# NirajNair/vector-indexer

Hardware: AMD Instinct MI355X
Metric: QPS at recall@10>=0.95 (IVF search, SIFT1M-shaped) (higher is better)
Workload: dtype f32; 1 GPU; IVF search N=1000000 D=128 nlist=4096 nprobe=32 k=10 nq/step=10000 (BASELINE configs[1]); nprobe=32, index_centroids=4094, parallelism=1 GPU

## Files before the change

### vector-indexer_amd/csrc/mfma_bf16.hpp

```cpp
#pragma once
#include <hip/hip_runtime.h>

#include <cmath>
#include <cstdint>

namespace vi {

typedef __bf16 bf16x8 __attribute__((ext_vector_type(8)));
typedef float f32x16 __attribute__((ext_vector_type(16)));
typedef __attribute__((address_space(3))) void *lds_ptr_t;

__device__ __forceinline__ float min3_raw(float a, float b, float c) {
  float d;
  asm("v_min3_f32 %0, %1, %2, %3" : "=v"(d) : "v"(a), "v"(b), "v"(c));
  return d;
}
__device__ __forceinline__ float opaque_neg_inf() {
  float v;
  asm("v_mov_b32 %0, 0xff800000" : "=v"(v));
  return v;
}
__device__ __forceinline__ void tile_min_level1(const f32x16 &a, float ninf, float (&p)[8]) {
#pragma unroll
  for (int i = 0; i < 8; ++i) p[i] = __builtin_amdgcn_fmed3f(ninf, a[2 * i], a[2 * i + 1]);
}
__device__ __forceinline__ float tile_min_level2(const float (&p)[8]) {
  const float m0 = min3_raw(p[0], p[1], p[2]), m1 = min3_raw(p[3], p[4], p[5]), m2 = min3_raw(p[6], p[7], p[7]);
  return min3_raw(m0, m1, m2);
}
__device__ __forceinline__ float tile_min(const f32x16 &a) {
  float p[8];
  tile_min_level1(a, opaque_neg_inf(), p);
  return tile_min_level2(p);
}
#define VI_TOP4(v)                             \
  {                                            \
    T3 = __builtin_amdgcn_fmed3f(T2, T3, v);   \
    T2 = __builtin_amdgcn_fmed3f(T1, T2, v);   \
    T1 = __builtin_amdgcn_fmed3f(T0, T1, v);   \
    T0 = min3_raw(T0, v, v);                   \
  }

__device__ __forceinline__ uint32_t bf16_rn(float x) {
  const uint32_t b = __float_as_uint(x);
  return (b + 0x7FFFu + ((b >> 16) & 1u)) >> 16;
}
__device__ __forceinline__ void split_pair(float x0, float x1, uint32_t &hi, uint32_t &lo) {
  const uint32_t h0 = bf16_rn(x0), h1 = bf16_rn(x1);
  const float r0 = x0 - __uint_as_float(h0 << 16), r1 = x1 - __uint_as_float(h1 << 16);
  hi = h0 | (h1 << 16);
  lo = bf16_rn(r0) | (bf16_rn(r1) << 16);
}
__device__ __forceinline__ void split8(const float4 &lo4, const float4 &hi4, float scale, uint4 &hi, uint4 &lo) {
  split_pair(scale * lo4.x, scale * lo4.y, hi.x, lo.x);
  split_pair(scale * lo4.z, scale * lo4.w, hi.y, lo.y);
  split_pair(scale * hi4.x, scale * hi4.y, hi.z, lo.z);
  split_pair(scale * hi4.z, scale * hi4.w, hi.w, lo.w);
}

template <int NG, int WAVES = 4>
__device__ __forceinline__ void tile_dma_image(float *tile, const float4 *src, const float *xn, int wave, int lane) {
#pragma unroll
  for (int i = 0; i < 2 * NG / WAVES; ++i) {
    const int piece = wave + WAVES * i;
    __builtin_amdgcn_global_load_lds(src + piece * 64 + lane, (lds_ptr_t)(tile + piece * 256), 16, 0, 0);
  }
  if (wave == 0) __builtin_amdgcn_global_load_lds(xn + lane, (lds_ptr_t)(tile + 2 * NG * 256), 4, 0, 0);
}

__device__ __forceinline__ void glds16_asm(const void *gsrc, float *lds_dst) {
  unsigned keep;
  const unsigned dst = (unsigned)__builtin_amdgcn_readfirstlane((int)(size_t)(lds_ptr_t)lds_dst);
  asm volatile("s_mov_b32 %0, m0\n\ts_mov_b32 m0, %2\n\ts_nop 0\n\tglobal_load_lds_dwordx4 %1, off\n\ts_mov_b32 m0, %0"
               : "=&s"(keep) : "v"(gsrc), "s"(dst) : "memory");
}
__device__ __forceinline__ void glds16_at(const void *gsrc, unsigned lds_addr) {
  unsigned keep;
  const unsigned dst = (unsigned)__builtin_amdgcn_readfirstlane((int)lds_addr);
  asm volatile("s_mov_b32 %0, m0\n\ts_mov_b32 m0, %2\n\ts_nop 0\n\tglobal_load_lds_dwordx4 %1, off\n\ts_mov_b32 m0, %0"
               : "=&s"(keep) : "v"(gsrc), "s"(dst) : "memory");
}
__device__ __forceinline__ void glds4_at(const void *gsrc, unsigned lds_addr) {
  unsigned keep;
  const unsigned dst = (unsigned)__builtin_amdgcn_readfirstlane((int)lds_addr);
  asm volatile("s_mov_b32 %0, m0\n\ts_mov_b32 m0, %2\n\ts_nop 0\n\tglobal_load_lds_dword %1, off\n\ts_mov_b32 m0, %0"
               : "=&s"(keep) : "v"(gsrc), "s"(dst) : "memory");
}
__device__ __forceinline__ void glds4_asm(const void *gsrc, float *lds_dst) {
  unsigned keep;
  const unsigned dst = (unsigned)__builtin_amdgcn_readfirstlane((int)(size_t)(lds_ptr_t)lds_dst);
  asm volatile("s_mov_b32 %0, m0\n\ts_mov_b32 m0, %2\n\ts_nop 0\n\tglobal_load_lds_dword %1, off\n\ts_mov_b32 m0, %0"
               : "=&s"(keep) : "v"(gsrc), "s"(dst) : "memory");
}

template <int NG, int WAVES = 4>
__device__ __forceinline__ void tile_dma_image_asm(float *tile, const float4 *src, const float *xn, int wave, int lane) {
#pragma unroll
  for (int i = 0; i < 2 * NG / WAVES; ++i) {
    const int piece = wave + WAVES * i;
    glds16_asm(src + piece * 64 + lane, tile + piece * 256);
  }
  if (wave == 0) glds4_asm(xn + lane, tile + 2 * NG * 256);
}

}
```

### vector-indexer_amd/csrc/rank_stream.hip

```cpp
#include <hip/hip_runtime.h>

#include <algorithm>
#include <cmath>
#include <cstdint>
#include <cstdio>
#include <cstdlib>
#include <vector>

#include "common.hpp"
#include "mfma_bf16.hpp"
#include "rank_stream.hpp"

namespace vi {
namespace {

constexpr int kWave = 64;
#ifdef VI_STREAM_PROF_BUILD
constexpr bool kStreamProf = true;
#else
constexpr bool kStreamProf = false;
#endif

typedef int i32x4 __attribute__((ext_vector_type(4)));
typedef int i32x16 __attribute__((ext_vector_type(16)));

template <int NC, int NA, class N4>
struct TileRegs {
  uint4 a[NC * NA];
  N4 n[4];
};

template <int IP, int NC, int NA, class N4, class N>
__device__ __forceinline__ void load_tile(TileRegs<NC, NA, N4> &t, const uint4 *img, const N *norm, uint32_t blk, uint32_t half, int il,
                                          int h) {
  const uint4 *ap = img + ((size_t)blk * (NC * 2 * IP) + h) * kWave + 32u * half + il;
#pragma unroll
  for (int c = 0; c < NC; ++c)
#pragma unroll
    for (int p = 0; p < NA; ++p) t.a[c * NA + p] = ap[(c * IP + p) * 2 * kWave];
  const N *np = norm + (size_t)blk * kWave + 32u * half + 4 * h;
#pragma unroll
  for (int q4 = 0; q4 < 4; ++q4) t.n[q4] = *reinterpret_cast<const N4 *>(np + 8 * q4);
}

template <int R>
struct StreamLayout {
  static constexpr int RP = R <= 2 ? 2 : R <= 4 ? 4 : R <= 8 ? 8 : R <= 16 ? 16 : 32;
  static_assert(R <= 32, "row too long");
  __device__ static __forceinline__ uint32_t swz(uint32_t pc, uint32_t q) {
    if constexpr (RP >= 16) return pc ^ (q & 15u);
    else return pc ^ ((q / (16u / RP)) & (uint32_t)(RP - 1));
  }
};

struct ItemRaw {
  uint4 d;
  uint32_t qid;
  uint32_t rec[2];
};
struct ItemRegs {
  uint32_t nqi, blk00, ntiles, rec0;
};

template <int NC, int NA, class N4>
__device__ __forceinline__ void tile_landed(const TileRegs<NC, NA, N4> &t) {
#pragma unroll
  for (int i = 0; i < NC * NA; ++i) asm volatile("" ::"v"(t.a[i].x), "v"(t.a[i].y), "v"(t.a[i].z), "v"(t.a[i].w));
#pragma unroll
  for (int q4 = 0; q4 < 4; ++q4) asm volatile("" ::"v"(t.n[q4].x), "v"(t.n[q4].y), "v"(t.n[q4].z), "v"(t.n[q4].w));
  __builtin_amdgcn_sched_barrier(0);
}

__device__ __forceinline__ void wait_vmcnt(uint32_t n) {
  switch (n) {
    case 1: asm volatile("s_waitcnt vmcnt(1)" ::: "memory"); break;
    case 2: asm volatile("s_waitcnt vmcnt(2)" ::: "memory"); break;
    case 3: asm volatile("s_waitcnt vmcnt(3)" ::: "memory"); break;
    case 4: asm volatile("s_waitcnt vmcnt(4)" ::: "memory"); break;
    case 5: asm volatile("s_waitcnt vmcnt(5)" ::: "memory"); break;
    case 6: asm volatile("s_waitcnt vmcnt(6)" ::: "memory"); break;
    case 7: asm volatile("s_waitcnt vmcnt(7)" ::: "memory"); break;
    case 8: asm volatile("s_waitcnt vmcnt(8)" ::: "memory"); break;
    default: asm volatile("s_waitcnt vmcnt(0)" ::: "memory"); break;
  }
}

__device__ __forceinline__ uint32_t queue_pop_asm(uint32_t *counter) {
  uint32_t ret;
  const uint32_t one = 1u;
  asm volatile("global_atomic_add %0, %1, %2, off sc0" : "=v"(ret) : "v"(counter), "v"(one) : "memory");
  return ret;
}

__device__ __forceinline__ void item_landed(const ItemRaw &r) {
  asm volatile("" ::"v"(r.d.x), "v"(r.d.y), "v"(r.d.z), "v"(r.d.w), "v"(r.qid), "v"(r.rec[0]), "v"(r.rec[1]));
  __builtin_amdgcn_sched_barrier(0);
}

__device__ __forceinline__ int tile_min_i32(const i32x16 &a) {
  int m[8];
#pragma unroll
  for (int i = 0; i < 8; ++i) m[i] = min(a[2 * i], a[2 * i + 1]);
  return min(min(min(m[0], m[1]), min(m[2], m[3])), min(min(m[4], m[5]), min(m[6], m[7])));
}


template <int RANK, bool QLO>
struct Bf16Form {
  static_assert(RANK == 2 || QLO, "bf16 x 3 needs the queries' lo plane");
  using Args = RankStreamArgs;
  using Norm4 = float4;
  using Frag = bf16x8;
  using Acc = f32x16;
  static constexpr int NA = RANK == 1 ? 2 : 1;
  static constexpr int NP = QLO ? 2 : 1;
  static constexpr int IP = 2;
  static constexpr bool kHooks = true;
  static constexpr int kRank = RANK;
  static constexpr bool kQlo = QLO;
  static constexpr const char *kName = "rank kernel";
  __device__ static __forceinline__ const float *norms(const Args &a) { return a.xnorm; }
  __device__ static __forceinline__ uint32_t xmode(const Args &a) { return a.xmode; }
  __device__ static __forceinline__ unsigned long long *prof(const Args &a) { return a.prof; }
  template <class T>
  __device__ static __forceinline__ Acc chunk(Acc acc, const T &t, int c, const Frag (&b)[NP]) {
    const bf16x8 ah = __builtin_bit_cast(bf16x8, t.a[c * NA]);
    acc = __builtin_amdgcn_mfma_f32_32x32x16_bf16(ah, b[0], acc, 0, 0, 0);
    if constexpr (QLO) acc = __builtin_amdgcn_mfma_f32_32x32x16_bf16(ah, b[NP - 1], acc, 0, 0, 0);
    if constexpr (RANK == 1) {
      const bf16x8 al = __builtin_bit_cast(bf16x8, t.a[c * NA + 1]);
      acc = __builtin_amdgcn_mfma_f32_32x32x16_bf16(al, b[0], acc, 0, 0, 0);
    }
    return acc;
  }
  __device__ static __forceinline__ float minimum(const Acc &acc) { return tile_min(acc); }
};

struct I8Form {
  using Args = RankStreamI8Args;
  using Norm4 = int4;
  using Frag = i32x4;
  using Acc = i32x16;
  static constexpr int NA = 1, NP = 1, IP = 1;
  static constexpr bool kHooks = false;
  static constexpr const char *kName = "int8 rank kernel";
  __device__ static __forceinline__ const int *norms(const Args &a) { return a.hnorm; }
  __device__ static __forceinline__ uint32_t xmode(const Args &) { return 0u; }
  __device__ static __forceinline__ unsigned long long *prof(const Args &) { return nullptr; }
  template <class T>
  __device__ static __forceinline__ Acc chunk(Acc acc, const T &t, int c, const Frag (&b)[NP]) {
    return __builtin_amdgcn_mfma_i32_32x32x32_i8(__builtin_bit_cast(i32x4, t.a[c]), b[0], acc, 0, 0, 0);
  }
  __device__ static __forceinline__ float minimum(const Acc &acc) { return (float)(2 * tile_min_i32(acc)); }
};

template <class F, int NC, int NU>
struct StreamShape {
  static constexpr int GQ = 32 * NU;
  using L = StreamLayout<2 * NC * F::NP>;
  static constexpr int IMG = GQ * L::RP * 16;
  static constexpr bool DB = IMG <= 32 * 1024;
  static constexpr size_t kLds = (size_t)IMG * (DB ? 2 : 1) + 2 * (size_t)NU * 1024 + 16;
};

template <class F, int NC, int NU>
__device__ __forceinline__ void rank_stream_body(typename F::Args a) {
  using S = StreamShape<F, NC, NU>;
  using L = typename S::L;
  using Tile = TileRegs<NC, F::NA, typename F::Norm4>;
  using Frag = typename F::Frag;
  constexpr int NP = F::NP;
  constexpr int GQ = S::GQ;
  constexpr int NR = NU / 4;
  constexpr int RP = L::RP;
  constexpr int RPI = 64 / RP;
  constexpr int IPW = GQ * RP / 256;
  constexpr int IMG = S::IMG;
  constexpr bool DB = S::DB;
  extern __shared__ __attribute__((aligned(16))) float s_mem[];
  float *s_T = s_mem + (DB ? 2 : 1) * (IMG / 4);
  uint32_t *s_idx = reinterpret_cast<uint32_t *>(s_T + 2 * 4 * NU * kWave);
  const int lane = threadIdx.x & (kWave - 1), wave = threadIdx.x >> 6;
  const int j = lane & 31, h = lane >> 5;
  const unsigned lds_q = (unsigned)(size_t)(lds_ptr_t)s_mem;
  auto load = [&](Tile &t, uint32_t blk, uint32_t half) { load_tile<F::IP>(t, a.img, F::norms(a), blk, half, j, h); };

  auto request_item = [&](uint32_t it, ItemRaw &r) {
    r.d = make_uint4(0u, 0u, 0u, 0u); r.qid = ~0u; r.rec[0] = ~0u; r.rec[1] = ~0u;
    if (it >= a.nitems) return;
    r.d = a.sdesc[it];
    if ((uint32_t)lane < (uint32_t)(GQ / 4)) r.qid = a.qcol[(size_t)it * GQ + (uint32_t)wave * (GQ / 4) + (uint32_t)lane];
#pragma unroll
    for (int k = 0; k < NR; ++k) r.rec[k] = a.grec[(size_t)it * GQ + 32u * ((uint32_t)wave + 4u * k) + (uint32_t)j];
  };
  auto decode_item = [&](const ItemRaw &r) {
    ItemRegs o;
    o.nqi = (uint32_t)__builtin_amdgcn_readfirstlane((int)r.d.x);
    o.blk00 = (uint32_t)__builtin_amdgcn_readfirstlane((int)r.d.y);
    o.ntiles = (uint32_t)__builtin_amdgcn_readfirstlane((int)r.d.z);
    o.rec0 = (uint32_t)__builtin_amdgcn_readfirstlane((int)r.d.w);
    return o;
  };
  auto gather = [&](uint32_t buf, uint32_t nq_item, uint32_t my_qid) {
    if (F::xmode(a) & 32u) return;
    uint32_t lo = (uint32_t)lane;
    asm volatile("" : "+v"(lo));
    uint32_t qids[IPW];
#pragma unroll
    for (int i = 0; i < IPW; ++i) qids[i] = (uint32_t)__shfl((int)my_qid, (int)(RPI * i + lo / RP));
#pragma unroll
    for (int i = 0; i < IPW; ++i) {
      const uint32_t row0 = (uint32_t)wave * (GQ / 4) + (uint32_t)(RPI * i);
      if (row0 < nq_item) {
        const uint32_t pc = L::swz(lo % RP, row0 + lo / RP);
        if (qids[i] != ~0u && pc < 2u * NC * NP)
          glds16_at(a.qimg + (size_t)qids[i] * (NC * 2 * F::IP) + pc, lds_q + buf * (uint32_t)IMG + row0 * RP * 16u);
      }
    }
  };

  const unsigned long long rt_begin = F::prof(a) ? __builtin_amdgcn_s_memrealtime() : 0ull;
  constexpr uint32_t kQueues = 8;
  auto queue_range = [&](uint32_t q, uint32_t &lo, uint32_t &hi) {
    lo = (uint32_t)(((uint64_t)a.nitems * q) / kQueues);
    hi = (uint32_t)(((uint64_t)a.nitems * (q + 1)) / kQueues);
  };
  uint32_t my_queue = blockIdx.x % kQueues;
  auto resolve = [&](uint32_t popped) {
    for (uint32_t tries = 0; tries < kQueues; ++tries) {
      uint32_t lo, hi;
      queue_range(my_queue, lo, hi);
      if (popped < hi - lo) return lo + popped;
      my_queue = (my_queue + 1) % kQueues;
      if (tries + 1 < kQueues) popped = atomicAdd(a.queue + 32 * my_queue, 1u);
    }
    return a.nitems;
  };
  const bool fixed = (F::xmode(a) & 64u) != 0u;
  if (threadIdx.x == 0) {
#pragma unroll
    for (uint32_t k = 0; k < 2; ++k) s_idx[k] = fixed ? blockIdx.x + k * gridDim.x : resolve(atomicAdd(a.queue + 32 * my_queue, 1u));
  }
  __syncthreads();
  uint32_t cur = (uint32_t)__builtin_amdgcn_readfirstlane((int)s_idx[0]), nxt = (uint32_t)__builtin_amdgcn_readfirstlane((int)s_idx[1]);
  ItemRaw rc, rn;
  request_item(cur, rc);
  request_item(nxt, rn);
  ItemRegs ic = decode_item(rc);
  Tile ta, tb;
  if ((uint32_t)wave < ic.ntiles) load(ta, ic.blk00 + ((uint32_t)wave >> 1), (uint32_t)wave & 1u);
  gather(0u, ic.nqi, rc.qid);
  asm volatile("s_waitcnt vmcnt(0)" ::: "memory");
  __syncthreads();
  tile_landed(ta);

  unsigned long long pt[16] = {0, 0, 0, 0, 0, 0, 0, 0, 0, 0, 0, 0, 0, 0, 0, 0};
  const bool prof = kStreamProf && F::prof(a) != nullptr && wave == 0;
  unsigned long long tk = prof ? __builtin_amdgcn_s_memtime() : 0ull;
  const unsigned long long tk_begin = tk;
  auto lap = [&](int slot) {
    if (prof) {
      const unsigned long long now = __builtin_amdgcn_s_memtime();
      pt[slot] += now - tk;
      tk = now;
    }
  };
  uint32_t buf = 0;
  uint32_t par = 0;
  uint32_t n_items = 0;
  const uint32_t lane_row = ((uint32_t)j * RP + L::swz(0u, (uint32_t)j)) * 16u;
  while (cur < a.nitems) {
    uint32_t after = ~0u;
    ItemRegs in{0u, 0u, 0u, 0u};
    auto last_step = [&](Tile &spare) {
      in = decode_item(rn);
      if ((uint32_t)wave < in.ntiles) load(spare, in.blk00 + ((uint32_t)wave >> 1), (uint32_t)wave & 1u);
      if (threadIdx.x == 0) after = fixed ? nxt + gridDim.x : queue_pop_asm(a.queue + 32 * my_queue);
      if (DB) gather(buf ^ 1u, in.nqi, rn.qid);
    };
    const uint32_t nqi = ic.nqi, nu = (ic.nqi + 31u) >> 5, ntiles = ic.ntiles, blk00 = ic.blk00;
    const char *img_at = reinterpret_cast<const char *>(s_mem) + (DB ? buf * (uint32_t)IMG : 0u);
    auto frag = [&](int c, int p, int u) {
      const uint32_t pc = (uint32_t)(p * 2 * NC + 2 * c) + (uint32_t)h;
      return __builtin_bit_cast(Frag, *reinterpret_cast<const uint4 *>(img_at + ((lane_row ^ (pc << 4)) + (uint32_t)(32 * u * RP * 16))));
    };

    float T[NU];
    float4 pend[NU];
#pragma unroll
    for (int u = 0; u < NU; ++u) {
      T[u] = INFINITY;
      pend[u] = make_float4(INFINITY, INFINITY, INFINITY, INFINITY);
    }
    const uint32_t bi = ic.rec0 * (2u * GQ) + (uint32_t)GQ * (uint32_t)h + (uint32_t)j;

    constexpr int kPF = 4;
    auto step = [&](const Tile &t, uint32_t i, bool last) {
      typename F::Acc nrm;
#pragma unroll
      for (int q4 = 0; q4 < 4; ++q4) {
        nrm[4 * q4 + 0] = t.n[q4].x; nrm[4 * q4 + 1] = t.n[q4].y; nrm[4 * q4 + 2] = t.n[q4].z; nrm[4 * q4 + 3] = t.n[q4].w;
      }
      Frag ring[kPF][NP];
      auto fetch = [&](int s) {
        const int u = (s / NC) < NU - 1 ? (s / NC) : NU - 1, c = s % NC;
#pragma unroll
        for (int p = 0; p < NP; ++p) ring[s % kPF][p] = frag(c, p, u);
      };
#pragma unroll
      for (int s0 = 0; s0 < kPF; ++s0) fetch(s0);
      const uint32_t ci = i & 3u;
#pragma unroll
      for (int u = 0; u < NU; ++u) {
        if ((uint32_t)u < nu) {
          typename F::Acc acc = nrm;
#pragma unroll
          for (int c = 0; c < NC; ++c) {
            const int sp = u * NC + c;
            __builtin_amdgcn_sched_barrier(0);
            acc = F::chunk(acc, t, c, ring[sp % kPF]);
            __builtin_amdgcn_sched_barrier(0);
            fetch(sp + kPF);
          }
          if (!(F::xmode(a) & 2u)) {
            const float m = F::minimum(acc);
            T[u] = min3_raw(T[u], m, m);
            pend[u].x = ci == 0u ? m : pend[u].x;
            pend[u].y = ci == 1u ? m : pend[u].y;
            pend[u].z = ci == 2u ? m : pend[u].z;
            pend[u].w = ci == 3u ? m : pend[u].w;
          }
        }
      }
      if (ci == 3u || last) {
        const uint32_t rt = (i >> 2) * 4u + (uint32_t)wave;
#pragma unroll
        for (int u = 0; u < NU; ++u) {
          if ((uint32_t)u < nu) {
            if (32u * u + (uint32_t)j < nqi && !(F::xmode(a) & 8u)) a.brec[(size_t)bi + 32u * u + (2u * GQ) * rt] = pend[u];
            pend[u] = make_float4(INFINITY, INFINITY, INFINITY, INFINITY);
          }
        }
      }
    };

    const bool restage = !(F::xmode(a) & 1u);
    bool prepared = false, next_in_tb = false;
    for (uint32_t i = 0;; i += 2) {
      const uint32_t t0 = 4u * i + (uint32_t)wave;
      if (t0 >= ntiles || (F::xmode(a) & 16u)) break;
      const uint32_t t1 = t0 + 4u, t2 = t0 + 8u;
      tile_landed(ta);
      item_landed(rn);
      if constexpr (F::kHooks) {
        if (t1 < ntiles && restage) load(tb, blk00 + (t1 >> 1), t1 & 1u);
        if (t1 >= ntiles) { last_step(tb); prepared = true; next_in_tb = true; }
      } else {
        if (t1 < ntiles) load(tb, blk00 + (t1 >> 1), t1 & 1u);
        else { last_step(tb); prepared = true; next_in_tb = true; }
      }
      step(ta, i, t1 >= ntiles);
      if (t1 >= ntiles) break;
      tile_landed(tb);
      item_landed(rn);
      if constexpr (F::kHooks) {
        if (t2 < ntiles && restage) load(ta, blk00 + (t2 >> 1), t2 & 1u);
        if (t2 >= ntiles) { last_step(ta); prepared = true; }
      } else {
        if (t2 < ntiles) load(ta, blk00 + (t2 >> 1), t2 & 1u);
        else { last_step(ta); prepared = true; }
      }
      step(tb, i + 1u, t2 >= ntiles);
    }
    if (!prepared) last_step(ta);
    const uint32_t young_stores = (ntiles > (uint32_t)wave && !(F::xmode(a) & (8u | 16u))) ? nu : 0u;

    lap(0);
    if (!DB) __syncthreads();
    lap(1);
    float *s_Tk = s_T + par * (4 * NU * kWave);
#pragma unroll
    for (int u = 0; u < NU; ++u)
      if ((uint32_t)u < nu) s_Tk[(wave * NU + u) * kWave + lane] = T[u];
    lap(8);
    if (!DB) gather(0u, in.nqi, rn.qid);
    lap(9);
    if (DB) wait_vmcnt(young_stores);
    else asm volatile("s_waitcnt vmcnt(0)" ::: "memory");
    if (threadIdx.x == 0) s_idx[par] = fixed ? after : resolve(after);
    lap(10);
    __syncthreads();
    lap(2);
    if (next_in_tb) ta = tb;
    asm volatile("" ::"v"(rc.rec[0]), "v"(rc.rec[1]));
    tile_landed(ta);
    __builtin_amdgcn_sched_barrier(0);
#pragma unroll
    for (int r = 0; r < NR; ++r) {
      const uint32_t u = (uint32_t)wave + 4u * r;
      if (u < nu) {
        float v0 = s_Tk[(0 * NU + u) * kWave + lane], v1 = s_Tk[(1 * NU + u) * kWave + lane];
        float v2 = s_Tk[(2 * NU + u) * kWave + lane], v3 = s_Tk[(3 * NU + u) * kWave + lane];
        auto cx = [](float &x, float &y) { const float lo = fminf(x, y), hi = fmaxf(x, y); x = lo; y = hi; };
        cx(v0, v1); cx(v2, v3); cx(v0, v2); cx(v1, v3); cx(v1, v2);
        if (rc.rec[r] != ~0u) a.gval[rc.rec[r] + (uint32_t)h] = make_float4(v0, v1, v2, v3);
      }
    }
    lap(11);
    cur = nxt;
    nxt = (uint32_t)__builtin_amdgcn_readfirstlane((int)s_idx[par]);
    par ^= 1u;
    ic = in;
    rc = rn;
    buf ^= 1u;
    lap(12);
    request_item(nxt, rn);
    lap(3);
    pt[4] += 1;
    ++n_items;
  }
  if (unsigned long long *pr = F::prof(a)) {
    if (threadIdx.x == 0) {
      pr[32 + 4 * blockIdx.x + 0] = rt_begin;
      pr[32 + 4 * blockIdx.x + 1] = __builtin_amdgcn_s_memrealtime();
      pr[32 + 4 * blockIdx.x + 2] = n_items;
    }
  }
  if (prof && lane == 0) {
    unsigned long long *pr = F::prof(a);
    pt[7] = __builtin_amdgcn_s_memtime() - tk_begin;
#pragma unroll
    for (int k = 0; k < 13; ++k) atomicAdd(pr + k, pt[k]);
    atomicMax(pr + 13, pt[7]);
    atomicAdd(pr + 14, pt[4] ? 1ull : 0ull);
    atomicMax(pr + 15, pt[4]);
    pr[32 + 4 * blockIdx.x + 3] = pt[0];
    atomicMin(pr + 16, tk_begin);
    atomicMax(pr + 17, tk_begin);
    atomicMax(pr + 18, tk_begin + pt[7]);
  }
}

template <int NC, int RANK, bool QLO, int NU>
__global__ void __launch_bounds__(256, 2) rank_stream_kernel(RankStreamArgs a) { rank_stream_body<Bf16Form<RANK, QLO>, NC, NU>(a); }

template <int NC, int NU>
__global__ void __launch_bounds__(256, 2) rank_stream_i8_kernel(RankStreamI8Args a) { rank_stream_body<I8Form, NC, NU>(a); }

template <class F, int NC, int NU>
vi_status launch_one(void (*kernel)(typename F::Args), const typename F::Args &a, uint32_t nitems, hipStream_t st) {
  constexpr size_t lds = StreamShape<F, NC, NU>::kLds;
  constexpr int kMaxDev = 64;
  static uint32_t cus_of[kMaxDev];
  int dev = 0;
  VI_HIP(hipGetDevice(&dev));
  if (dev < 0 || dev >= kMaxDev) return fail(VI_ERR_DEVICE, "device ordinal %d out of range", dev);
  uint32_t cus = __atomic_load_n(&cus_of[dev], __ATOMIC_ACQUIRE);
  if (cus == 0) {
    if (hipFuncSetAttribute((const void *)kernel, hipFuncAttributeMaxDynamicSharedMemorySize, (int)lds) != hipSuccess)
      return fail(VI_ERR_DEVICE, "cannot reserve %zu bytes of LDS for the %s", lds, F::kName);
    int n = 0;
    if (hipDeviceGetAttribute(&n, hipDeviceAttributeMultiprocessorCount, dev) != hipSuccess || n <= 0) n = 256;
    cus = (uint32_t)n;
    __atomic_store_n(&cus_of[dev], cus, __ATOMIC_RELEASE);
  }
  uint32_t per_cu = lds > 80 * 1024 ? 1u : 2u;
  if (const char *e = getenv("VI_STREAM_WGS_PER_CU")) per_cu = (uint32_t)std::max(1, atoi(e));
  const uint32_t grid = std::min(nitems, per_cu * cus);
  if constexpr (F::kHooks) {
    if (a.prof) {
      int nb = -1;
      (void)hipOccupancyMaxActiveBlocksPerMultiprocessor(&nb, (const void *)kernel, 256, lds);
      fprintf(stderr, "rank_stream<%d,%d,%d,%d>: lds %zu B, occupancy %d workgroups per CU, grid %u\n", NC, F::kRank, (int)F::kQlo, NU, lds,
              nb, grid);
    }
  }
  hipLaunchKernelGGL(kernel, dim3(grid), dim3(256), lds, st, a);
  VI_HIP(hipGetLastError());
  return VI_OK;
}

template <int NC>
vi_status launch_nc(const RankStreamArgs &a, uint32_t nitems, int rank_mode, bool qlo, uint32_t gq, hipStream_t st) {
  if (rank_mode != 2) return fail(VI_ERR_OTHER, "the streaming rank kernel is built for bf16-exact lists only");
  if (gq == 256) {
    if (!qlo) return launch_one<Bf16Form<2, false>, NC, 8>(rank_stream_kernel<NC, 2, false, 8>, a, nitems, st);
    return launch_one<Bf16Form<2, true>, NC, 8>(rank_stream_kernel<NC, 2, true, 8>, a, nitems, st);
  }
  if (!qlo) return launch_one<Bf16Form<2, false>, NC, 4>(rank_stream_kernel<NC, 2, false, 4>, a, nitems, st);
  return launch_one<Bf16Form<2, true>, NC, 4>(rank_stream_kernel<NC, 2, true, 4>, a, nitems, st);
}

template <int NC>
vi_status launch_nc_i8(const RankStreamI8Args &a, uint32_t nitems, uint32_t gq, hipStream_t st) {
  if (gq == 256) return launch_one<I8Form, NC, 8>(rank_stream_i8_kernel<NC, 8>, a, nitems, st);
  return launch_one<I8Form, NC, 4>(rank_stream_i8_kernel<NC, 4>, a, nitems, st);
}
}

vi_status launch_rank_stream(const RankStreamArgs &a, uint32_t nc, uint32_t nitems, int rank_mode, bool qlo, uint32_t gq, hipStream_t st) {
  if (nitems == 0) return VI_OK;
  switch (nc) {
    case 1: return launch_nc<1>(a, nitems, rank_mode, qlo, gq, st);
    case 2: return launch_nc<2>(a, nitems, rank_mode, qlo, gq, st);
    case 3: return launch_nc<3>(a, nitems, rank_mode, qlo, gq, st);
    case 4: return launch_nc<4>(a, nitems, rank_mode, qlo, gq, st);
    case 5: return launch_nc<5>(a, nitems, rank_mode, qlo, gq, st);
    case 6: return launch_nc<6>(a, nitems, rank_mode, qlo, gq, st);
    case 7: return launch_nc<7>(a, nitems, rank_mode, qlo, gq, st);
    case 8: return launch_nc<8>(a, nitems, rank_mode, qlo, gq, st);
    default: return fail(VI_ERR_OTHER, "unsupported dimension for the streaming rank kernel");
  }
}

vi_status launch_rank_stream_i8(const RankStreamI8Args &a, uint32_t nc32, uint32_t nitems, uint32_t gq, hipStream_t st) {
  if (nitems == 0) return VI_OK;
  switch (nc32) {
    case 1: return launch_nc_i8<1>(a, nitems, gq, st);
    case 2: return launch_nc_i8<2>(a, nitems, gq, st);
    case 3: return launch_nc_i8<3>(a, nitems, gq, st);
    case 4: return launch_nc_i8<4>(a, nitems, gq, st);
    default: return fail(VI_ERR_OTHER, "unsupported dimension for the int8 rank kernel");
  }
}

vi_status print_rank_stream_profile(const uint64_t *prof_dev, const char *dump_path, hipStream_t st) {
  constexpr int kTotals = 32, kWorkgroups = (kRankStreamProfWords - kTotals) / 4;
  uint64_t h[24];
  VI_HIP(hipMemcpyAsync(h, prof_dev, sizeof(h), hipMemcpyDeviceToHost, st));
  VI_HIP(hipStreamSynchronize(st));
  fprintf(stderr, "rank_stream wave-0 ticks (100 MHz) summed over workgroups: multiply %llu (of which waiting for tiles %llu) "
          "end-of-item wait %llu gather %llu merge %llu | items %llu steps %llu | loop total %llu\n",
          (unsigned long long)h[0], (unsigned long long)h[6], (unsigned long long)h[1], (unsigned long long)h[2],
          (unsigned long long)h[3], (unsigned long long)h[4], (unsigned long long)h[5], (unsigned long long)h[7]);
  if (dump_path) {
    std::vector<uint64_t> w(4 * kWorkgroups);
    VI_HIP(hipMemcpy(w.data(), prof_dev + kTotals, w.size() * sizeof(uint64_t), hipMemcpyDeviceToHost));
    if (FILE *f = fopen(dump_path, "w")) {
      uint64_t base = ~0ull;
      for (int i = 0; i < kWorkgroups; ++i) if (w[4 * i + 1]) base = std::min(base, w[4 * i]);
      for (int i = 0; i < kWorkgroups; ++i)
        if (w[4 * i + 1]) fprintf(f, "%d %llu %llu %llu\n", i, (unsigned long long)(w[4 * i] - base), (unsigned long long)(w[4 * i + 1] - base),
                                  (unsigned long long)w[4 * i + 2]);
      fclose(f);
    }
  }
  fprintf(stderr, "   loops entered over %llu ticks, last exit %llu ticks after the first entry\n", (unsigned long long)(h[17] - h[16]),
          (unsigned long long)(h[18] - h[16]));
  fprintf(stderr, "   longest workgroup loop %llu ticks, workgroups with items %llu, most items in one %llu\n", (unsigned long long)h[13],
          (unsigned long long)h[14], (unsigned long long)h[15]);
  fprintf(stderr, "   after B1: T+idx %llu, DMA issue %llu, vmcnt(0) %llu, B2 %llu | after B2: merge+stores %llu, idx read %llu, load_item %llu\n",
          (unsigned long long)h[8], (unsigned long long)h[9], (unsigned long long)h[10], (unsigned long long)h[2],
          (unsigned long long)h[11], (unsigned long long)h[12], (unsigned long long)h[3]);
  return VI_OK;
}

}
```

Before: 27.32 million queries/s.

## Stage work-item metadata through LDS and emit tile loads as inline asm

Per-item descriptors, query ids and record indices are now DMA'd into per-wave LDS slots with global_load_lds, no longer held in VGPRs, so gather and record lookups read from LDS. Tile loads become inline-asm global_load_dwordx4 with immediate offsets, and explicit vmcnt waits are placed so stores can stay in flight while the next tile lands. The aim is to cut register pressure and the conservative waits on item registers, at the cost of more LDS and hand-managed memory-counter ordering that is fragile if the counts are wrong.

```diff
diff --git a/vector-indexer_amd/csrc/mfma_bf16.hpp b/vector-indexer_amd/csrc/mfma_bf16.hpp
--- a/vector-indexer_amd/csrc/mfma_bf16.hpp
+++ b/vector-indexer_amd/csrc/mfma_bf16.hpp
@@ -93,6 +93,12 @@
                : "=&s"(keep) : "v"(gsrc), "s"(dst) : "memory");
 }
 
+template <int OFF, class V>
+__device__ __forceinline__ void gload16_asm(V &dst, const void *gsrc) {
+  static_assert(sizeof(V) == 16 && OFF >= -4096 && OFF < 4096, "one dwordx4, immediate offset");
+  asm volatile("global_load_dwordx4 %0, %1, off offset:%2" : "+v"(dst) : "v"(gsrc), "i"(OFF) : "memory");
+}
+
 template <int NG, int WAVES = 4>
 __device__ __forceinline__ void tile_dma_image_asm(float *tile, const float4 *src, const float *xn, int wave, int lane) {
 #pragma unroll
diff --git a/vector-indexer_amd/csrc/rank_stream.hip b/vector-indexer_amd/csrc/rank_stream.hip
--- a/vector-indexer_amd/csrc/rank_stream.hip
+++ b/vector-indexer_amd/csrc/rank_stream.hip
@@ -5,6 +5,7 @@
 #include <cstdint>
 #include <cstdio>
 #include <cstdlib>
+#include <utility>
 #include <vector>
 
 #include "common.hpp"
@@ -20,27 +21,37 @@
 #else
 constexpr bool kStreamProf = false;
 #endif
+#ifdef VI_STREAM_ABLATE_STORES_BUILD
+constexpr bool kAblateRecordStores = true;
+#else
+constexpr bool kAblateRecordStores = false;
+#endif
 
 typedef int i32x4 __attribute__((ext_vector_type(4)));
 typedef int i32x16 __attribute__((ext_vector_type(16)));
+typedef uint32_t u32x4 __attribute__((ext_vector_type(4)));
+typedef float f32x4 __attribute__((ext_vector_type(4)));
 
 template <int NC, int NA, class N4>
 struct TileRegs {
-  uint4 a[NC * NA];
+  u32x4 a[NC * NA];
   N4 n[4];
 };
 
+template <int IP, int NA, class T, int... I>
+__device__ __forceinline__ void load_tile_pieces(T &t, const char *ap, std::integer_sequence<int, I...>) {
+  (gload16_asm<((I / NA * IP + I % NA) * 2 * kWave * 16) % 4096>(t.a[I], ap + ((I / NA * IP + I % NA) * 2 * kWave * 16) / 4096 * 4096), ...);
+}
 template <int IP, int NC, int NA, class N4, class N>
 __device__ __forceinline__ void load_tile(TileRegs<NC, NA, N4> &t, const uint4 *img, const N *norm, uint32_t blk, uint32_t half, int il,
                                           int h) {
   const uint4 *ap = img + ((size_t)blk * (NC * 2 * IP) + h) * kWave + 32u * half + il;
-#pragma unroll
-  for (int c = 0; c < NC; ++c)
-#pragma unroll
-    for (int p = 0; p < NA; ++p) t.a[c * NA + p] = ap[(c * IP + p) * 2 * kWave];
+  load_tile_pieces<IP, NA>(t, reinterpret_cast<const char *>(ap), std::make_integer_sequence<int, NC * NA>());
   const N *np = norm + (size_t)blk * kWave + 32u * half + 4 * h;
-#pragma unroll
-  for (int q4 = 0; q4 < 4; ++q4) t.n[q4] = *reinterpret_cast<const N4 *>(np + 8 * q4);
+  gload16_asm<0>(t.n[0], np);
+  gload16_asm<32>(t.n[1], np);
+  gload16_asm<64>(t.n[2], np);
+  gload16_asm<96>(t.n[3], np);
 }
 
 template <int R>
@@ -53,36 +64,47 @@
   }
 };
 
-struct ItemRaw {
-  uint4 d;
-  uint32_t qid;
-  uint32_t rec[2];
+struct ItemSlot {
+  static constexpr uint32_t kDesc = 0;
+  static constexpr uint32_t kQid = 4;
+  static constexpr uint32_t kRec = 68;
+  __host__ __device__ static constexpr uint32_t words(int nr) { return kRec + 64u * (uint32_t)nr; }
 };
 struct ItemRegs {
   uint32_t nqi, blk00, ntiles, rec0;
 };
 
 template <int NC, int NA, class N4>
-__device__ __forceinline__ void tile_landed(const TileRegs<NC, NA, N4> &t) {
-#pragma unroll
-  for (int i = 0; i < NC * NA; ++i) asm volatile("" ::"v"(t.a[i].x), "v"(t.a[i].y), "v"(t.a[i].z), "v"(t.a[i].w));
-#pragma unroll
-  for (int q4 = 0; q4 < 4; ++q4) asm volatile("" ::"v"(t.n[q4].x), "v"(t.n[q4].y), "v"(t.n[q4].z), "v"(t.n[q4].w));
+__device__ __forceinline__ void tile_arrived(TileRegs<NC, NA, N4> &t) {
+#pragma unroll
+  for (int i = 0; i < NC * NA; ++i) asm volatile("" : "+v"(t.a[i]));
+#pragma unroll
+  for (int q4 = 0; q4 < 4; ++q4) asm volatile("" : "+v"(t.n[q4]));
   __builtin_amdgcn_sched_barrier(0);
 }
 
 __device__ __forceinline__ void wait_vmcnt(uint32_t n) {
-  switch (n) {
-    case 1: asm volatile("s_waitcnt vmcnt(1)" ::: "memory"); break;
-    case 2: asm volatile("s_waitcnt vmcnt(2)" ::: "memory"); break;
-    case 3: asm volatile("s_waitcnt vmcnt(3)" ::: "memory"); break;
-    case 4: asm volatile("s_waitcnt vmcnt(4)" ::: "memory"); break;
-    case 5: asm volatile("s_waitcnt vmcnt(5)" ::: "memory"); break;
-    case 6: asm volatile("s_waitcnt vmcnt(6)" ::: "memory"); break;
-    case 7: asm volatile("s_waitcnt vmcnt(7)" ::: "memory"); break;
-    case 8: asm volatile("s_waitcnt vmcnt(8)" ::: "memory"); break;
-    default: asm volatile("s_waitcnt vmcnt(0)" ::: "memory"); break;
-  }
+  const uint32_t s = (uint32_t)__builtin_amdgcn_readfirstlane((int)n);
+  asm volatile(
+      "s_cmp_eq_u32 %0, 1\n\ts_cbranch_scc1 1f\n\t"
+      "s_cmp_eq_u32 %0, 2\n\ts_cbranch_scc1 2f\n\t"
+      "s_cmp_eq_u32 %0, 3\n\ts_cbranch_scc1 3f\n\t"
+      "s_cmp_eq_u32 %0, 4\n\ts_cbranch_scc1 4f\n\t"
+      "s_cmp_eq_u32 %0, 5\n\ts_cbranch_scc1 5f\n\t"
+      "s_cmp_eq_u32 %0, 6\n\ts_cbranch_scc1 6f\n\t"
+      "s_cmp_eq_u32 %0, 7\n\ts_cbranch_scc1 7f\n\t"
+      "s_cmp_eq_u32 %0, 8\n\ts_cbranch_scc1 8f\n\t"
+      "s_waitcnt vmcnt(0)\n\ts_branch 9f\n"
+      "1:\n\ts_waitcnt vmcnt(1)\n\ts_branch 9f\n"
+      "2:\n\ts_waitcnt vmcnt(2)\n\ts_branch 9f\n"
+      "3:\n\ts_waitcnt vmcnt(3)\n\ts_branch 9f\n"
+      "4:\n\ts_waitcnt vmcnt(4)\n\ts_branch 9f\n"
+      "5:\n\ts_waitcnt vmcnt(5)\n\ts_branch 9f\n"
+      "6:\n\ts_waitcnt vmcnt(6)\n\ts_branch 9f\n"
+      "7:\n\ts_waitcnt vmcnt(7)\n\ts_branch 9f\n"
+      "8:\n\ts_waitcnt vmcnt(8)\n"
+      "9:"
+      :: "s"(s) : "scc", "memory");
 }
 
 __device__ __forceinline__ uint32_t queue_pop_asm(uint32_t *counter) {
@@ -92,9 +114,10 @@
   return ret;
 }
 
-__device__ __forceinline__ void item_landed(const ItemRaw &r) {
-  asm volatile("" ::"v"(r.d.x), "v"(r.d.y), "v"(r.d.z), "v"(r.d.w), "v"(r.qid), "v"(r.rec[0]), "v"(r.rec[1]));
-  __builtin_amdgcn_sched_barrier(0);
+template <int NC, int NA, class N4>
+__device__ __forceinline__ void tile_wait(TileRegs<NC, NA, N4> &t, uint32_t younger) {
+  wait_vmcnt(younger);
+  tile_arrived(t);
 }
 
 __device__ __forceinline__ int tile_min_i32(const i32x16 &a) {
@@ -109,7 +132,7 @@
 struct Bf16Form {
   static_assert(RANK == 2 || QLO, "bf16 x 3 needs the queries' lo plane");
   using Args = RankStreamArgs;
-  using Norm4 = float4;
+  using Norm4 = f32x4;
   using Frag = bf16x8;
   using Acc = f32x16;
   static constexpr int NA = RANK == 1 ? 2 : 1;
@@ -138,7 +161,7 @@
 
 struct I8Form {
   using Args = RankStreamI8Args;
-  using Norm4 = int4;
+  using Norm4 = i32x4;
   using Frag = i32x4;
   using Acc = i32x16;
   static constexpr int NA = 1, NP = 1, IP = 1;
@@ -160,7 +183,8 @@
   using L = StreamLayout<2 * NC * F::NP>;
   static constexpr int IMG = GQ * L::RP * 16;
   static constexpr bool DB = IMG <= 32 * 1024;
-  static constexpr size_t kLds = (size_t)IMG * (DB ? 2 : 1) + 2 * (size_t)NU * 1024 + 16;
+  static constexpr uint32_t kSlot = ItemSlot::words(NU / 4);
+  static constexpr size_t kLds = (size_t)IMG * (DB ? 2 : 1) + 2 * (size_t)NU * 1024 + 16 + 4 * 2 * 4 * (size_t)kSlot;
 };
 
 template <class F, int NC, int NU>
@@ -183,31 +207,36 @@
   const int lane = threadIdx.x & (kWave - 1), wave = threadIdx.x >> 6;
   const int j = lane & 31, h = lane >> 5;
   const unsigned lds_q = (unsigned)(size_t)(lds_ptr_t)s_mem;
+  constexpr uint32_t kSlot = S::kSlot;
+  uint32_t *s_item = s_idx + 4 + (uint32_t)wave * (2u * kSlot);
+  const unsigned lds_item = (unsigned)(size_t)(lds_ptr_t)s_item;
   auto load = [&](Tile &t, uint32_t blk, uint32_t half) { load_tile<F::IP>(t, a.img, F::norms(a), blk, half, j, h); };
 
-  auto request_item = [&](uint32_t it, ItemRaw &r) {
-    r.d = make_uint4(0u, 0u, 0u, 0u); r.qid = ~0u; r.rec[0] = ~0u; r.rec[1] = ~0u;
+  auto request_item = [&](uint32_t it, uint32_t p) {
     if (it >= a.nitems) return;
-    r.d = a.sdesc[it];
-    if ((uint32_t)lane < (uint32_t)(GQ / 4)) r.qid = a.qcol[(size_t)it * GQ + (uint32_t)wave * (GQ / 4) + (uint32_t)lane];
-#pragma unroll
-    for (int k = 0; k < NR; ++k) r.rec[k] = a.grec[(size_t)it * GQ + 32u * ((uint32_t)wave + 4u * k) + (uint32_t)j];
+    const unsigned at = lds_item + p * (4u * kSlot);
+    if (lane == 0) glds16_at(a.sdesc + it, at + 4u * ItemSlot::kDesc);
+    if ((uint32_t)lane < (uint32_t)(GQ / 4)) glds4_at(a.qcol + (size_t)it * GQ + (uint32_t)wave * (GQ / 4) + (uint32_t)lane, at + 4u * ItemSlot::kQid);
+#pragma unroll
+    for (int k = 0; k < NR; ++k) glds4_at(a.grec + (size_t)it * GQ + 32u * ((uint32_t)wave + 4u * k) + (uint32_t)j, at + 4u * (ItemSlot::kRec + 64u * k));
   };
-  auto decode_item = [&](const ItemRaw &r) {
-    ItemRegs o;
-    o.nqi = (uint32_t)__builtin_amdgcn_readfirstlane((int)r.d.x);
-    o.blk00 = (uint32_t)__builtin_amdgcn_readfirstlane((int)r.d.y);
-    o.ntiles = (uint32_t)__builtin_amdgcn_readfirstlane((int)r.d.z);
-    o.rec0 = (uint32_t)__builtin_amdgcn_readfirstlane((int)r.d.w);
+  auto decode_item = [&](uint32_t it, uint32_t p) {
+    ItemRegs o{0u, 0u, 0u, 0u};
+    if (it >= a.nitems) return o;
+    const uint4 d = *reinterpret_cast<const uint4 *>(s_item + p * kSlot + ItemSlot::kDesc);
+    o.nqi = (uint32_t)__builtin_amdgcn_readfirstlane((int)d.x);
+    o.blk00 = (uint32_t)__builtin_amdgcn_readfirstlane((int)d.y);
+    o.ntiles = (uint32_t)__builtin_amdgcn_readfirstlane((int)d.z);
+    o.rec0 = (uint32_t)__builtin_amdgcn_readfirstlane((int)d.w);
     return o;
   };
-  auto gather = [&](uint32_t buf, uint32_t nq_item, uint32_t my_qid) {
+  auto gather = [&](uint32_t buf, uint32_t nq_item, uint32_t p) {
     if (F::xmode(a) & 32u) return;
     uint32_t lo = (uint32_t)lane;
     asm volatile("" : "+v"(lo));
     uint32_t qids[IPW];
 #pragma unroll
-    for (int i = 0; i < IPW; ++i) qids[i] = (uint32_t)__shfl((int)my_qid, (int)(RPI * i + lo / RP));
+    for (int i = 0; i < IPW; ++i) qids[i] = s_item[p * kSlot + ItemSlot::kQid + (uint32_t)(RPI * i) + lo / RP];
 #pragma unroll
     for (int i = 0; i < IPW; ++i) {
       const uint32_t row0 = (uint32_t)wave * (GQ / 4) + (uint32_t)(RPI * i);
@@ -232,7 +261,10 @@
       queue_range(my_queue, lo, hi);
       if (popped < hi - lo) return lo + popped;
       my_queue = (my_queue + 1) % kQueues;
-      if (tries + 1 < kQueues) popped = atomicAdd(a.queue + 32 * my_queue, 1u);
+      if (tries + 1 < kQueues) {
+        popped = queue_pop_asm(a.queue + 32 * my_queue);
+        asm volatile("s_waitcnt vmcnt(0)" : "+v"(popped)::"memory");
+      }
     }
     return a.nitems;
   };
@@ -243,16 +275,16 @@
   }
   __syncthreads();
   uint32_t cur = (uint32_t)__builtin_amdgcn_readfirstlane((int)s_idx[0]), nxt = (uint32_t)__builtin_amdgcn_readfirstlane((int)s_idx[1]);
-  ItemRaw rc, rn;
-  request_item(cur, rc);
-  request_item(nxt, rn);
-  ItemRegs ic = decode_item(rc);
-  Tile ta, tb;
+  request_item(cur, 0u);
+  request_item(nxt, 1u);
+  asm volatile("s_waitcnt vmcnt(0)" ::: "memory");
+  ItemRegs ic = decode_item(cur, 0u);
+  Tile ta{}, tb{};
   if ((uint32_t)wave < ic.ntiles) load(ta, ic.blk00 + ((uint32_t)wave >> 1), (uint32_t)wave & 1u);
-  gather(0u, ic.nqi, rc.qid);
+  gather(0u, ic.nqi, 0u);
   asm volatile("s_waitcnt vmcnt(0)" ::: "memory");
   __syncthreads();
-  tile_landed(ta);
+  tile_arrived(ta);
 
   unsigned long long pt[16] = {0, 0, 0, 0, 0, 0, 0, 0, 0, 0, 0, 0, 0, 0, 0, 0};
   const bool prof = kStreamProf && F::prof(a) != nullptr && wave == 0;
@@ -272,11 +304,12 @@
   while (cur < a.nitems) {
     uint32_t after = ~0u;
     ItemRegs in{0u, 0u, 0u, 0u};
-    auto last_step = [&](Tile &spare) {
-      in = decode_item(rn);
+    auto last_step = [&](Tile &spare, bool at_once) {
+      if (at_once) asm volatile("s_waitcnt vmcnt(0)" ::: "memory");
+      in = decode_item(nxt, par ^ 1u);
       if ((uint32_t)wave < in.ntiles) load(spare, in.blk00 + ((uint32_t)wave >> 1), (uint32_t)wave & 1u);
       if (threadIdx.x == 0) after = fixed ? nxt + gridDim.x : queue_pop_asm(a.queue + 32 * my_queue);
-      if (DB) gather(buf ^ 1u, in.nqi, rn.qid);
+      if (DB) gather(buf ^ 1u, in.nqi, par ^ 1u);
     };
     const uint32_t nqi = ic.nqi, nu = (ic.nqi + 31u) >> 5, ntiles = ic.ntiles, blk00 = ic.blk00;
     const char *img_at = reinterpret_cast<const char *>(s_mem) + (DB ? buf * (uint32_t)IMG : 0u);
@@ -295,6 +328,7 @@
     const uint32_t bi = ic.rec0 * (2u * GQ) + (uint32_t)GQ * (uint32_t)h + (uint32_t)j;
 
     constexpr int kPF = 4;
+    const bool rec_stores = !kAblateRecordStores && !(F::xmode(a) & 8u);
     auto step = [&](const Tile &t, uint32_t i, bool last) {
       typename F::Acc nrm;
 #pragma unroll
@@ -337,7 +371,7 @@
 #pragma unroll
         for (int u = 0; u < NU; ++u) {
           if ((uint32_t)u < nu) {
-            if (32u * u + (uint32_t)j < nqi && !(F::xmode(a) & 8u)) a.brec[(size_t)bi + 32u * u + (2u * GQ) * rt] = pend[u];
+            if (32u * u + (uint32_t)j < nqi && rec_stores) a.brec[(size_t)bi + 32u * u + (2u * GQ) * rt] = pend[u];
             pend[u] = make_float4(INFINITY, INFINITY, INFINITY, INFINITY);
           }
         }
@@ -350,30 +384,30 @@
       const uint32_t t0 = 4u * i + (uint32_t)wave;
       if (t0 >= ntiles || (F::xmode(a) & 16u)) break;
       const uint32_t t1 = t0 + 4u, t2 = t0 + 8u;
-      tile_landed(ta);
-      item_landed(rn);
       if constexpr (F::kHooks) {
         if (t1 < ntiles && restage) load(tb, blk00 + (t1 >> 1), t1 & 1u);
-        if (t1 >= ntiles) { last_step(tb); prepared = true; next_in_tb = true; }
+        if (t1 >= ntiles) { last_step(tb, i == 0u); prepared = true; next_in_tb = true; }
       } else {
         if (t1 < ntiles) load(tb, blk00 + (t1 >> 1), t1 & 1u);
-        else { last_step(tb); prepared = true; next_in_tb = true; }
+        else { last_step(tb, i == 0u); prepared = true; next_in_tb = true; }
       }
       step(ta, i, t1 >= ntiles);
       if (t1 >= ntiles) break;
-      tile_landed(tb);
-      item_landed(rn);
+      asm volatile("s_waitcnt vmcnt(0)" ::: "memory");
+      tile_arrived(tb);
       if constexpr (F::kHooks) {
         if (t2 < ntiles && restage) load(ta, blk00 + (t2 >> 1), t2 & 1u);
-        if (t2 >= ntiles) { last_step(ta); prepared = true; }
+        if (t2 >= ntiles) { last_step(ta, false); prepared = true; }
       } else {
         if (t2 < ntiles) load(ta, blk00 + (t2 >> 1), t2 & 1u);
-        else { last_step(ta); prepared = true; }
+        else { last_step(ta, false); prepared = true; }
       }
       step(tb, i + 1u, t2 >= ntiles);
-    }
-    if (!prepared) last_step(ta);
-    const uint32_t young_stores = (ntiles > (uint32_t)wave && !(F::xmode(a) & (8u | 16u))) ? nu : 0u;
+      if (t2 >= ntiles) break;
+      tile_wait(ta, ((i & 2u) && rec_stores) ? nu : 0u);
+    }
+    if (!prepared) last_step(ta, true);
+    const uint32_t young_stores = (ntiles > (uint32_t)wave && !kAblateRecordStores && !(F::xmode(a) & (8u | 16u))) ? nu : 0u;
 
     lap(0);
     if (!DB) __syncthreads();
@@ -383,7 +417,7 @@
     for (int u = 0; u < NU; ++u)
       if ((uint32_t)u < nu) s_Tk[(wave * NU + u) * kWave + lane] = T[u];
     lap(8);
-    if (!DB) gather(0u, in.nqi, rn.qid);
+    if (!DB) gather(0u, in.nqi, par ^ 1u);
     lap(9);
     if (DB) wait_vmcnt(young_stores);
     else asm volatile("s_waitcnt vmcnt(0)" ::: "memory");
@@ -391,10 +425,9 @@
     lap(10);
     __syncthreads();
     lap(2);
+    tile_arrived(ta);
+    tile_arrived(tb);
     if (next_in_tb) ta = tb;
-    asm volatile("" ::"v"(rc.rec[0]), "v"(rc.rec[1]));
-    tile_landed(ta);
-    __builtin_amdgcn_sched_barrier(0);
 #pragma unroll
     for (int r = 0; r < NR; ++r) {
       const uint32_t u = (uint32_t)wave + 4u * r;
@@ -403,7 +436,8 @@
         float v2 = s_Tk[(2 * NU + u) * kWave + lane], v3 = s_Tk[(3 * NU + u) * kWave + lane];
         auto cx = [](float &x, float &y) { const float lo = fminf(x, y), hi = fmaxf(x, y); x = lo; y = hi; };
         cx(v0, v1); cx(v2, v3); cx(v0, v2); cx(v1, v3); cx(v1, v2);
-        if (rc.rec[r] != ~0u) a.gval[rc.rec[r] + (uint32_t)h] = make_float4(v0, v1, v2, v3);
+        const uint32_t rec = s_item[par * kSlot + ItemSlot::kRec + 64u * r + (uint32_t)lane];
+        if (rec != ~0u) a.gval[rec + (uint32_t)h] = make_float4(v0, v1, v2, v3);
       }
     }
     lap(11);
@@ -411,10 +445,9 @@
     nxt = (uint32_t)__builtin_amdgcn_readfirstlane((int)s_idx[par]);
     par ^= 1u;
     ic = in;
-    rc = rn;
     buf ^= 1u;
     lap(12);
-    request_item(nxt, rn);
+    request_item(nxt, par ^ 1u);
     lap(3);
     pt[4] += 1;
     ++n_items;
```

Result: no change. 27.59 million queries/s, median of 4 (+1.0%).
